# cv3vpl-lab/cylinder-pose-estimation

Hardware: AMD Instinct MI355X
Metric: frames/sec (grid-detect + cylinder fit) on 1920x1200 batch (higher is better)
Workload: dtype f64

## Files before the change

cylinder-pose-estimation_amd/csrc/masks.hip:

```cpp
#include "cpe_dev.h"

namespace cpe {

namespace {

struct W3 { unsigned long long a, b, c; };
template <int K> __device__ __forceinline__ W3 w3_up(const W3 &v, unsigned long long fill)
{
    W3 r;
    r.a = (v.a >> K) | (v.b << (64 - K));
    r.b = (v.b >> K) | (v.c << (64 - K));
    r.c = (v.c >> K) | (fill << (64 - K));
    return r;
}
template <int K> __device__ __forceinline__ W3 w3_down(const W3 &v, unsigned long long fill)
{
    W3 r;
    r.c = (v.c << K) | (v.b >> (64 - K));
    r.b = (v.b << K) | (v.a >> (64 - K));
    r.a = (v.a << K) | (fill >> (64 - K));
    return r;
}
__device__ __forceinline__ W3 w3_and(const W3 &x, const W3 &y) { return W3{x.a & y.a, x.b & y.b, x.c & y.c}; }
__device__ __forceinline__ W3 w3_or(const W3 &x, const W3 &y) { return W3{x.a | y.a, x.b | y.b, x.c | y.c}; }
// ... 921 lines not shown
{
    const int f = blockIdx.y;
    if (st[f].status != CPE_ST_OK) return;
    __shared__ unsigned long long s_win[BW_ROWS * 64];
    __shared__ float s_pts[SEG_LPW][2 * MAXVS];
    const int ncomp = min(*root_counter(st[f], list), MAXROOTS);
    if (threadIdx.x >= SEG_LPW) return;
    for (int k = blockIdx.x * SEG_LPW + threadIdx.x; k < ncomp; k += gridDim.x * SEG_LPW) {
    const int root = roots[(size_t)f * MAXROOTS + k];
    if (!comp_is_external(outside + f * plane_words, w, root, window_rect(st, f, WIN_REGION, h, w).x0)) continue;
    BitWin nz{bit_plane(base_bits, f, h, w), w, h, s_win + threadIdx.x};
    float *pts = s_pts[threadIdx.x];
    SegVisitor sv{pts, MAXVS};
    if (!trace_border(nz, root % w, root / w, false, sv, 8 * (w + h) + (1 << 20))) { set_overflow(st[f], OVF_TRACE); continue; }
    const int n = sv.n;
    if (n < MINV || n > MAXVS) continue;
    float mx = 0, my = 0;
    for (int i = 0; i < n; i++) { mx += pts[2 * i]; my += pts[2 * i + 1]; }
    mx = mx / (float)n; my = my / (float)n;
    double ax = 0, ay = 0;
    for (int i = 0; i < n; i++) { ax += (double)(pts[2 * i] - mx); ay += (double)(pts[2 * i + 1] - my); }
    ax /= n; ay /= n;
    double sxx = 0, sxy = 0, syy = 0;
    for (int i = 0; i < n; i++) {
        double dx = (double)(pts[2 * i] - mx) - ax, dy = (double)(pts[2 * i + 1] - my) - ay;
        sxx += dx * dx; sxy += dx * dy; syy += dy * dy;
    }
    double fct = 1.0 / (n - 1);
    sxx *= fct; sxy *= fct; syy *= fct;
    double wv[2], V[4];
    eig2_lapack(sxx, sxy, sxy, syy, wv, V);
    int kk = wv[1] > wv[0] ? 1 : 0;
    double ux = V[0 + kk], uy = V[2 + kk];
    int imin = 0, imax = 0;
    double pmin = 0, pmax = 0;
    for (int i = 0; i < n; i++) {
        double pr = (double)(pts[2 * i] - mx) * ux + (double)(pts[2 * i + 1] - my) * uy;
        if (i == 0 || pr < pmin) { pmin = pr; imin = i; }
        if (i == 0 || pr > pmax) { pmax = pr; imax = i; }
    }
    float p1x = pts[2 * imin], p1y = pts[2 * imin + 1], p2x = pts[2 * imax], p2y = pts[2 * imax + 1];
    float dx = p2x - p1x, dy = p2y - p1y;
    float length = (float)hypot((double)dx, (double)dy);
    if (length < 1e-8) continue;
    float at = (float)atan2((double)dy, (double)dx);
    float deg = at * (float)(180.0 / 3.14159265358979323846);
    int q = atomicAdd(&st[f].n_seg[which], 1);
    if (q >= MAXSEG) { set_overflow(st[f], OVF_SEGS); continue; }
    SegRec &r = segs[(size_t)f * MAXSEG + q];
    r.p1x = p1x; r.p1y = p1y; r.p2x = p2x; r.p2y = p2y; r.angle = -deg; r.len = length; r.valid = 1;
    }
}

__global__ __launch_bounds__(256) void k_seg_global(FrameState *__restrict__ st, int which, const SegRec *__restrict__ segs)
{
    const int f = blockIdx.x, t = threadIdx.x;
    __shared__ float s_lo, s_hi;
    __shared__ unsigned int s_len;
    const int nv = min(st[f].n_seg[which], MAXSEG);
    const SegRec *S = segs + (size_t)f * MAXSEG;
    if (t == 0) { s_lo = 0; s_hi = 0; s_len = 0; }
    __syncthreads();
    const int k_hi = nv / 2, k_lo = (nv & 1) ? nv / 2 : nv / 2 - 1;
    for (int i = t; i < nv; i += 256) {
        float ai = S[i].angle;
        int rank = 0;
        for (int j = 0; j < nv; j++) {
            float aj = S[j].angle;
            rank += (aj < ai || (aj == ai && j < i)) ? 1 : 0;
        }
        if (rank == k_lo) s_lo = ai;
        if (rank == k_hi) s_hi = ai;
        atomicMax(&s_len, __float_as_uint(S[i].len));
    }
    __syncthreads();
    if (t == 0) {
        st[f].gang[which] = (nv & 1) ? s_hi : (float)(((double)s_lo + (double)s_hi) / 2.0);
        st[f].glen[which] = __uint_as_float(s_len);
    }
}

constexpr int EXP_MAXKS = 176;
constexpr int EXP_MAXKS_PLANE = 208;
template <int MAXKS>
__global__ __launch_bounds__(256) void k_seg_expand(const uint8_t *__restrict__ base, int h, int w, int which,
                                                    FrameState *__restrict__ st, const SegRec *__restrict__ segs,
                                                    uint8_t *__restrict__ exp, int fixed_ks)
{
    constexpr int EXP_REG = 15 + MAXKS + 2;
    __shared__ uint8_t dil[EXP_REG * EXP_REG];
    __shared__ short koff[4096][2];
    __shared__ short ppix[225][2];
    __shared__ int s_nk, s_np;
    const int f = blockIdx.y, t = threadIdx.x;
    FrameState &S = st[f];
    if (S.status != CPE_ST_OK) return;
    const int njobs = 2 * min(S.n_seg[which], MAXSEG);
    for (int job = blockIdx.x; job < njobs; job += gridDim.x) {
    const int seg = job >> 1, e = job & 1;
    const SegRec r = segs[(size_t)f * MAXSEG + seg];
    const float glen = S.glen[which], gang = S.gang[which];
    if ((double)r.len > 0.8 * (double)glen) continue;
    const int ks = fixed_ks > 0 ? fixed_ks : 91 + S.r0;
    if (ks > MAXKS) { if (t == 0) set_overflow(S, OVF_KERNEL); return; }
    __syncthreads();
    const float ak = fabsf(r.angle - gang) > 5.0f ? gang : r.angle;
    const int a = ks / 2, half = 7;
    const size_t N = (size_t)h * w;
    const uint8_t *bm = base + f * N;
    const int cx = (int)rint((double)(e ? r.p2x : r.p1x)), cy = (int)rint((double)(e ? r.p2y : r.p1y));
    const int x1 = max(cx - half, 0), x2 = min(cx + half + 1, w), y1 = max(cy - half, 0), y2 = min(cy + half + 1, h);
    if (t == 0) { s_nk = 0; s_np = 0; }
    __syncthreads();
    {
        const int c = ks / 2;
        double ar = (double)ak * 3.1415926535897932384626433832795 / 180.0;
        double alpha = cos(ar), beta = sin(ar);
        double M[6] = {alpha, beta, (1 - alpha) * c - beta * c, -beta, alpha, beta * c + (1 - alpha) * c};
        double D = M[0] * M[4] - M[1] * M[3];
        D = D != 0 ? 1. / D : 0;
        double A11 = M[4] * D, A22 = M[0] * D;
        double iM[6];
        iM[0] = A11; iM[1] = M[1] * (-D); iM[3] = M[3] * (-D); iM[4] = A22;
        double b1 = -iM[0] * M[2] - iM[1] * M[5];
        double b2 = -iM[3] * M[2] - iM[4] * M[5];
        iM[2] = b1; iM[5] = b2;
        for (int i = t; i < ks * ks; i += 256) {
            int y = i / ks, x = i - y * ks;
            int X0 = (int)rint((iM[1] * y + iM[2]) * 1024) + 512;
            int Y0 = (int)rint((iM[4] * y + iM[5]) * 1024) + 512;
            int adelta = (int)rint(iM[0] * x * 1024), bdelta = (int)rint(iM[3] * x * 1024);
            int X = (X0 + adelta) >> 10, Y = (Y0 + bdelta) >> 10;
            if (X >= 0 && X < ks && Y == c) {
                int q = atomicAdd(&s_nk, 1);
                if (q < 4096) { koff[q][0] = (short)(x - a); koff[q][1] = (short)(y - a); }
            }
        }
    }
    for (int i = t; i < 225; i += 256) {
        int py = y1 + i / 15, px = x1 + i % 15;
        if (py < y2 && px < x2 && bm[(size_t)py * w + px]) {
            int q = atomicAdd(&s_np, 1);
            ppix[q][0] = (short)px; ppix[q][1] = (short)py;
        }
    }
    const int bx1 = x1 - a - 1, by1 = y1 - a - 1;
    const int bw = (x2 - x1) + 2 * a + 2, bh = (y2 - y1) + 2 * a + 2;
    for (int i = t; i < bw * bh; i += 256) dil[i] = 0;
    __syncthreads();
    const int nk = min(s_nk, 4096), np = s_np;
    if (s_nk > 4096 && t == 0) set_overflow(S, OVF_EXPAND);
    for (int i = t; i < nk * np; i += 256) {
        int p = i / nk, k = i - p * nk;
        int xx = ppix[p][0] - koff[k][0], yy = ppix[p][1] - koff[k][1];
        if (xx >= 0 && xx < w && yy >= 0 && yy < h) dil[(yy - by1) * bw + (xx - bx1)] = 1;
    }
    __syncthreads();
    uint8_t *ex = exp + f * N;
    for (int i = t; i < bw * bh; i += 256) {
        int ly = i / bw, lx = i - ly * bw;
        int gy = by1 + ly, gx = bx1 + lx;
        if (gx < 0 || gx >= w || gy < 0 || gy >= h) continue;
        bool all = true;
        for (int dy = -1; dy <= 1 && all; dy++)
            for (int dx = -1; dx <= 1; dx++) {
                int yy = gy + dy, xx = gx + dx;
                if (yy < 0 || yy >= h || xx < 0 || xx >= w) continue;
                int ly2 = ly + dy, lx2 = lx + dx;
                bool v = (ly2 >= 0 && ly2 < bh && lx2 >= 0 && lx2 < bw) ? dil[ly2 * bw + lx2] != 0 : false;
                if (!v) { all = false; break; }
            }
        if (all) ex[(size_t)gy * w + gx] = 255;
    }
    }
}

__global__ void k_masks_reset(FrameState *st, int n)
{
    int f = blockIdx.x * blockDim.x + threadIdx.x;
    if (f >= n) return;
    FrameState &S = st[f];
    S.n_joints = 0; S.n_joints_all = 0; S.n_seg[0] = 0; S.n_seg[1] = 0;
    S.gang[0] = S.gang[1] = 0; S.glen[0] = S.glen[1] = 0;
    if (S.status == CPE_ST_NO_REGION) { S.r0 = 0; S.spot[0] = S.spot[1] = S.spot[2] = S.spot[3] = 0; }
    else if (S.status == CPE_ST_OK && S.spot_fail) S.status = CPE_ST_NO_SPOT;
}

inline unsigned grid1(size_t total) { return (unsigned)((total + 255) / 256); }

}


__global__ __launch_bounds__(256) void k_blur7_bgr(const uint8_t *__restrict__ bgr, int h, int w, int tiles_x, int tiles_y, Taps t,
                                                   const FrameState *__restrict__ st, uint8_t *__restrict__ dst)
{
    constexpr int R = 3, IW = BT_X + 2 * R, IH = BT_Y + 2 * R, PER = BT_X * BT_Y / 256;
    __shared__ uint8_t s_in[IH * IW];
    __shared__ uint16_t s_h[IH * BT_X];
    const int tid = threadIdx.x;
    const int tiles = tiles_x * tiles_y;
    const int f = blockIdx.x / tiles, tt = blockIdx.x - f * tiles;
    const int gx0 = (tt % tiles_x) * BT_X, gy0 = (tt / tiles_x) * BT_Y;
    const size_t N = (size_t)h * w;
    const FrameState &S = st[f];
    if (S.status != CPE_ST_OK) return;
    int half = (int)(S.r0 / 5.0);
    if (half < 3) half = 3;
    if (half > 10) half = half + 5;
    half = max(half, (int)(S.r0 / 4.5));
    const int m = half + 1;
    if (gx0 > S.rect[0] + S.rect[2] + m || gx0 + BT_X < S.rect[0] - m || gy0 > S.rect[1] + S.rect[3] + m || gy0 + BT_Y < S.rect[1] - m)
        return;
    const uint8_t *im = bgr + f * N * 3;
    uint32_t ch[PER][3];
    for (int c = 0; c < 3; c++) {
        for (int i = tid; i < IH * IW; i += 256) {
            int ry = i / IW, rx = i - ry * IW;
            s_in[i] = im[((size_t)reflect101(gy0 - R + ry, h) * w + reflect101(gx0 - R + rx, w)) * 3 + c];
        }
        __syncthreads();
        for (int i = tid; i < IH * BT_X; i += 256) {
            int ry = i / BT_X, rx = i - ry * BT_X;
            const uint8_t *p = &s_in[ry * IW + rx];
            int sacc = 0;
#pragma unroll
            for (int j = 0; j <= 2 * R; j++) sacc += t.k[j] * p[j];
            s_h[i] = (uint16_t)sacc;
        }
        __syncthreads();
#pragma unroll
        for (int q = 0; q < PER; q++) {
            const int i = tid + q * 256;
            int ry = i / BT_X, rx = i - ry * BT_X;
            const uint16_t *p = &s_h[ry * BT_X + rx];
            int sacc = 0;
#pragma unroll
            for (int j = 0; j <= 2 * R; j++) sacc += t.k[j] * (int)p[j * BT_X];
            ch[q][c] = (uint32_t)((sacc + (1 << (t.shift - 1))) >> t.shift);
        }
        __syncthreads();
    }
#pragma unroll
    for (int q = 0; q < PER; q++) {
        const int i = tid + q * 256;
        int ry = i / BT_X, rx = i - ry * BT_X;
        if (gy0 + ry < h && gx0 + rx < w)
            dst[f * N + (size_t)(gy0 + ry) * w + gx0 + rx] = (uint8_t)((ch[q][0] * 3735u + ch[q][1] * 19235u + ch[q][2] * 9798u + 16384u) >> 15);
    }
}

int blur7_bgr(const uint8_t *bgr, int n, int h, int w, const FrameState *st, uint8_t *dst, hipStream_t s)
{
    Taps t7 = {{2, 7, 14, 18, 14, 7, 2}, 3, 12};
    CPE_LAUNCH_BEGIN();
    const int tiles_x = (w + BT_X - 1) / BT_X, tiles_y = (h + BT_Y - 1) / BT_Y;
// ... 24 lines not shown
        if (lds64 <= 96 * 1024) {
            const int bands = (h + 63) / 64;
            CPE_KLAUNCH(k_open20_joints<64>, dim3((unsigned)(n * bands)), dim3(256), lds64, s, (const uint8_t *)B.binary, h, w, bands,
                        B.hmask, B.vmask, B.joints_mask, B.jbits);
        } else {
            CPE_CHECK_ARG(lds32 <= 160 * 1024, "joints_mask_stage: frame too wide (%d columns)", w);
            const int bands = (h + 31) / 32;
            CPE_KLAUNCH(k_open20_joints<32>, dim3((unsigned)(n * bands)), dim3(256), lds32, s, (const uint8_t *)B.binary, h, w, bands,
                        B.hmask, B.vmask, B.joints_mask, B.jbits);
        }
    }
    CPE_CHECK_LAUNCH("joints_mask_stage");
    int rc;
    if ((rc = ccl_components(B.joints_mask, B.jbits, n, h, w, 0, WIN_FRAME, B.lab_p, B.roots_p, ROOTS_JOINTS, st, s)) != CPE_OK) return rc;
    const size_t fl_words = (size_t)h * ((w + 63) / 64);
    return outside_flood(B.joints_mask, n, h, w, st, WIN_FRAME, B.fl_j, B.fl_j + (size_t)n * fl_words, fl_words, s, B.jbits);
}

int spot_stage(const uint8_t *gray, int n, int h, int w, const MaskBuffers &B, FrameState *st, hipStream_t s, int planar)
{
    const size_t total = (size_t)h * w * n;
    int rc;
    CPE_LAUNCH_BEGIN();
    Taps t19 = {{1, 1, 3, 5, 10, 15, 20, 27, 30, 32, 30, 27, 20, 15, 10, 5, 3, 1, 1}, 9, 16};
    {
        const int tiles_x = (w + BT_X - 1) / BT_X, tiles_y = (h + BT_Y - 1) / BT_Y;
        CPE_CHECK_ARG(tiles_x <= 128 && (size_t)tiles_x * tiles_y <= (size_t)MAXROOTS * sizeof(int), "spot_stage: frame too large");
        uint8_t *flags = reinterpret_cast<uint8_t *>(B.roots_s);
        const size_t fstride = (size_t)MAXROOTS * sizeof(int);
        CPE_KLAUNCH(k_spot_scan, dim3((unsigned)(n * tiles_y)), dim3(256), 0, s, gray, h, w, tiles_x, tiles_y, st, flags, fstride);
        CPE_KLAUNCH(k_blur19_spot, dim3((unsigned)(n * tiles_y)), dim3(256), 0, s, gray, h, w, tiles_x, tiles_y, t19,
                    (const uint8_t *)flags, fstride, B.g19);
    }
    if ((rc = ccl_components(B.g19, nullptr, n, h, w, 240, WIN_SPOT, B.lab_s, B.roots_s, ROOTS_SPOT, st, s)) != CPE_OK) return rc;
    CPE_KLAUNCH(k_spot_area, dim3(4, n), dim3(64), 0, s, B.g19, h, w, B.roots_s, st, B.best_s);
    (void)hipMemsetAsync(B.cm, 255, total, s);
    CPE_KLAUNCH(k_spot_ellipse, dim3(n), dim3(64), 0, s, B.g19, n, h, w, B.best_s, st, B.verts, B.cm, planar);
    CPE_CHECK_LAUNCH("spot_stage");
    return CPE_OK;
}

int masks_stage(const uint8_t *gray, int n, int h, int w, const MaskBuffers &B, FrameState *st, hipStream_t s,
                const RegionSide *side, int planar, hipStream_t sj)
{
    const size_t total = (size_t)h * w * n;
    int rc;
    CPE_LAUNCH_BEGIN();
    CPE_KLAUNCH(k_masks_reset, dim3((n + 63) / 64), dim3(64), 0, s, st, n);
    const size_t fl_words = bit_plane_words(h, w);
    auto fl_plane = [&](int k) { return bit_plane(B.bits, (size_t)(2 + k) * n, h, w); };
    const bool jside = side && sj != s;
    if (jside) { (void)hipEventRecord(side->clahe_done, s); (void)hipStreamWaitEvent(sj, side->clahe_done, 0); }
    {
        hipStream_t q = jside ? sj : s;
        CPE_KLAUNCH(k_joint_centroids, dim3(frame_waves(n, 16, MAXROOTS / 64), n), dim3(64), 0, q, (const uint32_t *)B.jbits, h, w, B.roots_p, st, B.jtmp,
                    (const unsigned long long *)(B.fl_j + (size_t)n * h * ((w + 63) / 64)), (size_t)h * ((w + 63) / 64));
        CPE_KLAUNCH(k_joint_sort, dim3(n), dim3(256), 0, q, st, B.jtmp, B.joints);
    }
    const int rb_bands = (h + RB_R - 1) / RB_R;
    const size_t rb_lds = (size_t)2 * RB_ROWS * ((w + 63) / 64) * 8;
    CPE_CHECK_ARG(rb_lds <= 160 * 1024, "masks_stage: frame too wide (%d columns)", w);
    CPE_CHECK_HIP(hipFuncSetAttribute(reinterpret_cast<const void *>(&k_roi_base), hipFuncAttributeMaxDynamicSharedMemorySize, 160 * 1024));
    if (side) { (void)hipEventRecord(side->clahe_done, s); (void)hipStreamWaitEvent(side->s, side->clahe_done, 0); }
    for (int which = 0; which < 2; which++) {
        hipStream_t q = (which && side) ? side->s : s;
        const uint8_t *lm = which ? B.vmask : B.hmask;
        uint8_t *roi = which ? B.roi_v : B.roi_h;
        uint8_t *base = which ? B.base_v : B.base_h;
        uint8_t *exp = which ? B.exp_v : B.exp_h;
        uint8_t *tmp = which ? B.tmpA : B.tmpB;
        int *lab = which ? B.lab_s : B.lab, *roots = which ? B.roots_s : B.roots;
        const RootList list = which ? ROOTS_SPOT : ROOTS_MAIN;
        uint32_t *bits = reinterpret_cast<uint32_t *>(bit_plane(B.bits, which ? (size_t)n : 0, h, w));
        SegRec *segs = B.segs + (size_t)which * n * MAXSEG;
        CPE_KLAUNCH(k_roi_base, dim3((unsigned)(n * rb_bands)), dim3(256), rb_lds, q, lm, (const uint8_t *)B.cm, (const uint8_t *)B.mc,
                    h, w, rb_bands, (const FrameState *)st, roi, base, bits);
        if ((rc = ccl_components(base, bits, n, h, w, 0, WIN_REGION, lab, roots, list, st, q)) != CPE_OK) return rc;
        unsigned long long *fl_bg = fl_plane(2 + 2 * which), *fl_out = fl_plane(3 + 2 * which);
        if ((rc = outside_flood(base, n, h, w, st, WIN_REGION, fl_bg, fl_out, fl_words, q, bits)) != CPE_OK) return rc;
        if (planar) CPE_KLAUNCH((k_seg_trace<8, 700>), dim3(frame_waves(n, 32, 512), n), dim3(64), 0, q, (const uint32_t *)bits, h, w, which, (const int *)roots, list, st, segs, (const unsigned long long *)fl_out, fl_words);
        else CPE_KLAUNCH((k_seg_trace<5, 200>), dim3(frame_waves(n, 32, 512), n), dim3(64), 0, q, (const uint32_t *)bits, h, w, which, (const int *)roots, list, st, segs, (const unsigned long long *)fl_out, fl_words);
        CPE_KLAUNCH(k_seg_global, dim3(n), dim3(256), 0, q, st, which, (const SegRec *)segs);
        (void)hipMemsetAsync(tmp, 0, total, q);
        if (planar) CPE_KLAUNCH(k_seg_expand<EXP_MAXKS_PLANE>, dim3(frame_waves(n, 32, 256), n), dim3(256), 0, q, (const uint8_t *)base, h, w, which, st, (const SegRec *)segs, tmp, 201);
        else CPE_KLAUNCH(k_seg_expand<EXP_MAXKS>, dim3(frame_waves(n, 32, 256), n), dim3(256), 0, q, (const uint8_t *)base, h, w, which, st, (const SegRec *)segs, tmp, 0);
        CPE_KLAUNCH(k_or_and, dim3((unsigned)(((size_t)h * w + 16383) / 16384), n), dim3(256), 0, q, (const uint8_t *)tmp, (const uint8_t *)base,
                    (const uint8_t *)B.mc, h, w, (const FrameState *)st, exp);
        CPE_CHECK_LAUNCH("masks_stage expand");
        if ((rc = ccl_unions(exp, n, h, w, WIN_REGION, which ? B.lab_v : B.lab_h, st, q)) != CPE_OK) return rc;
    }
    if (side) { (void)hipEventRecord(side->traced, side->s); (void)hipStreamWaitEvent(s, side->traced, 0); }
    return CPE_OK;
}

}
```

cylinder-pose-estimation_amd/csrc/region.hip:

```cpp
#include "cpe_dev.h"
#include <stdlib.h>

namespace cpe {

namespace {

__constant__ uint8_t c_lab_l[256] = { 0, 1, 1, 2, 2, 3, 5, 5, 6, 7, 7, 8, 9, 9, 10, 11, 12, 12, 14, 15, 16, 17, 18, 19, 21, 23, 24, 25, 27, 27, 28, 30, 31, 33, 34, 35, 36, 38, 39, 40, 41, 42, 43, 45, 46, 47, 48, 50, 51, 52, 53, 54, 55, 57, 58, 59, 60, 61, 62, 63, 65, 66, 67, 68, 69, 70, 71, 73, 74, 75, 76, 77, 78, 79, 80, 82, 82, 83, 85, 86, 87, 88, 89, 90, 91, 92, 93, 94, 95, 97, 98, 99, 100, 101, 102, 103, 104, 105, 106, 107, 108, 109, 110, 111, 112, 113, 114, 115, 116, 117, 119, 119, 121, 122, 123, 124, 125, 126, 127, 128, 129, 130, 131, 132, 133, 134, 135, 136, 137, 138, 139, 140, 141, 142, 143, 144, 145, 146, 147, 148, 149, 150, 151, 152, 153, 154, 155, 156, 156, 157, 158, 159, 160, 161, 162, 163, 164, 165, 166, 167, 168, 169, 170, 171, 172, 173, 174, 175, 176, 177, 178, 179, 180, 180, 181, 182, 183, 184, 185, 186, 187, 188, 189, 190, 191, 192, 193, 194, 195, 196, 196, 197, 198, 199, 200, 201, 202, 203, 204, 205, 206, 207, 208, 208, 209, 210, 211, 212, 213, 214, 215, 216, 217, 218, 219, 219, 220, 221, 222, 223, 224, 225, 226, 227, 228, 228, 229, 230, 231, 232, 233, 234, 235, 236, 237, 237, 238, 239, 240, 241, 242, 243, 244, 245, 245, 246, 247, 248, 249, 250, 251, 252, 253, 253, 254, 255 };

__device__ __forceinline__ int sat_u8(int v) { return v < 0 ? 0 : (v > 255 ? 255 : v); }

struct ClaheGeom { int tilesX, tilesY, tw, th, eh, ew, clipLimit; float lutScale; };

constexpr int HIST_COPIES = 4;
__global__ __launch_bounds__(256) void k_clahe_hist(const uint8_t *__restrict__ gray, int n, int h, int w, ClaheGeom g,
                                                    int strips, unsigned int *__restrict__ hist, int lab_lut)
{
    __shared__ unsigned int sh[4 * 256 * HIST_COPIES];
    int b = blockIdx.x;
    int strip = b % strips; b /= strips;
    int tile = b % (g.tilesX * g.tilesY);
    int f = b / (g.tilesX * g.tilesY);
    int ty = tile / g.tilesX, tx = tile - ty * g.tilesX;
    for (int k = threadIdx.x; k < 4 * 256 * HIST_COPIES; k += 256) sh[k] = 0;
    __syncthreads();
// ... 557 lines not shown
}

constexpr int SEL_CAP = 256;
template <class Get>
__device__ double wave_select(Get get, int n, int k, int lane, double *s_buf , int *s_hist , int *s_cnt)
{
    double lo = -1e300, hi = 1e300;
    for (;;) {
        double mn = 1e300, mx = -1e300;
        int cnt = 0, below = 0;
        for (int i = lane; i < n; i += 64) {
            const double v = get(i);
            if (v < lo) below++;
            else if (v <= hi) { cnt++; mn = fmin(mn, v); mx = fmax(mx, v); }
        }
        for (int off = 32; off >= 1; off >>= 1) {
            mn = fmin(mn, __shfl_xor(mn, off, 64)); mx = fmax(mx, __shfl_xor(mx, off, 64));
            cnt += __shfl_xor(cnt, off, 64); below += __shfl_xor(below, off, 64);
        }
        const int kk = k - below;
        if (mx == mn) return mn;
        __syncthreads();
        if (cnt <= SEL_CAP) {
            if (lane == 0) *s_cnt = 0;
            __syncthreads();
            for (int i = lane; i < n; i += 64) {
                const double v = get(i);
                if (v >= lo && v <= hi) s_buf[atomicAdd(s_cnt, 1)] = v;
            }
            __syncthreads();
            double found = -1e300;
            for (int j = lane; j < cnt; j += 64) {
                const double x = s_buf[j];
                int less = 0, leq = 0;
                for (int q = 0; q < cnt; q++) { const double y = s_buf[q]; less += (y < x) ? 1 : 0; leq += (y <= x) ? 1 : 0; }
                if (less <= kk && kk < leq) found = x;
            }
            for (int off = 32; off >= 1; off >>= 1) found = fmax(found, __shfl_xor(found, off, 64));
            return found;
        }
        const double scale = 64.0 / (mx - mn);
        s_hist[lane] = 0;
        __syncthreads();
        for (int i = lane; i < n; i += 64) {
            const double v = get(i);
            if (v >= lo && v <= hi) atomicAdd(&s_hist[min(63, (int)((v - mn) * scale))], 1);
        }
        __syncthreads();
        const int hc = s_hist[lane];
        int incl = hc;
        for (int off = 1; off < 64; off <<= 1) { int tt = __shfl_up(incl, off, 64); if (lane >= off) incl += tt; }
        const int bstar = __popcll(__ballot(incl <= kk));
        double nlo = 1e300, nhi = -1e300;
        for (int i = lane; i < n; i += 64) {
            const double v = get(i);
            if (v >= lo && v <= hi && min(63, (int)((v - mn) * scale)) == bstar) { nlo = fmin(nlo, v); nhi = fmax(nhi, v); }
        }
        for (int off = 32; off >= 1; off >>= 1) { nlo = fmin(nlo, __shfl_xor(nlo, off, 64)); nhi = fmax(nhi, __shfl_xor(nhi, off, 64)); }
        lo = nlo; hi = nhi;
    }
}

template <class Get>
__device__ double wave_median(Get get, int n, int lane, double *s_buf, int *s_hist, int *s_cnt)
{
    const int k1 = (n - 1) / 2, k2 = n / 2;
    const double v1 = wave_select(get, n, k1, lane, s_buf, s_hist, s_cnt);
    double v2 = v1;
    if (k2 != k1) {
        int le = 0;
        double nxt = 1e300;
        for (int i = lane; i < n; i += 64) {
            const double v = get(i);
            if (v <= v1) le++;
            else nxt = fmin(nxt, v);
        }
        for (int off = 32; off >= 1; off >>= 1) { le += __shfl_xor(le, off, 64); nxt = fmin(nxt, __shfl_xor(nxt, off, 64)); }
        if (le <= k2) v2 = nxt;
    }
    return (v1 + v2) / 2.;
}

constexpr int MED_FAST = CH_DIRECT * CH_PTS;

__global__ __launch_bounds__(64) void k_blob_median(int part, int *__restrict__ sw, BlobRec *__restrict__ blobs_all,
                                                    const int *__restrict__ blob_d_all, double *__restrict__ dists_all,
                                                    const uint32_t *__restrict__ pool_all,
                                                    const unsigned short *__restrict__ blob_ch_all, FrameState *__restrict__ st,
                                                    int maxch, int maxdf)
{
    __shared__ double s_d[MED_FAST > SEL_CAP ? MED_FAST : SEL_CAP];
    __shared__ int s_ch[MAXCHAIN];
    __shared__ int s_hist[64];
    __shared__ int s_cnt;
    const int f = blockIdx.y, slot = blockIdx.z, lane = threadIdx.x;
    int *S = sw + (size_t)f * SW_STRIDE;
    const int nb = min(S[SW_NB + slot], MAXB);
    if (!part && blockIdx.x == 0 && lane == 0) S[SW_NA + slot] = nb;
    BlobRec *blobs = blobs_all + ((size_t)f * NTHR + slot) * MAXB;
    const int *blob_d = blob_d_all + ((size_t)f * NTHR + slot) * MAXB * 2;
    double *dists = dists_all + (size_t)f * NTHR * maxdf;
    const uint32_t *pool = pool_all + ((size_t)f * NTHR + slot) * maxch * 32;
    const unsigned short *blob_ch = blob_ch_all + ((size_t)f * NTHR + slot) * MAXB * CH_DIRECT;
    for (int bi = (part ? S[SW_NA + slot] : 0) + blockIdx.x; bi < nb; bi += gridDim.x) {
        const int code = blob_d[bi * 2], n = blob_d[bi * 2 + 1];
        if (code < 0 || n <= 0) continue;
        double r;
        if ((code & PTS_STORED) && n <= MED_FAST) {
            const double cx = blobs[bi].x, cy = blobs[bi].y;
            const int myid = lane < CH_DIRECT ? (int)blob_ch[bi * CH_DIRECT + lane] : 0;
            double v[MED_FAST / 64 + 1];
            double mn = 1e300, mx = -1.0;
#pragma unroll
            for (int m = 0; m < MED_FAST / 64 + 1; m++) {
                const int i = lane + 64 * m;
                const bool valid = i < n;
                const int c = __shfl(myid, valid ? i / CH_PTS : 0, 64);
                v[m] = -1.0;
                if (valid) {
                    const uint32_t p = pool[(size_t)c * 32 + i % CH_PTS];
                    const double dx = cx - (double)(int)(p & 0xFFFFu), dy = cy - (double)(int)(p >> 16);
                    v[m] = dx * dx + dy * dy;
                    mn = fmin(mn, v[m]); mx = fmax(mx, v[m]);
                }
            }
            for (int off = 32; off >= 1; off >>= 1) { mn = fmin(mn, __shfl_xor(mn, off, 64)); mx = fmax(mx, __shfl_xor(mx, off, 64)); }
            double res[2] = {mn, mn};
            if (mx > mn) {
                const double scale = 64.0 / (mx - mn);
                int bkt[MED_FAST / 64 + 1];
                __syncthreads();
                s_hist[lane] = 0;
                __syncthreads();
#pragma unroll
                for (int m = 0; m < MED_FAST / 64 + 1; m++) {
                    bkt[m] = -1;
                    if (v[m] >= 0.0) { bkt[m] = min(63, (int)((v[m] - mn) * scale)); atomicAdd(&s_hist[bkt[m]], 1); }
                }
                __syncthreads();
                const int hc = s_hist[lane];
                int incl = hc;
                for (int off = 1; off < 64; off <<= 1) { int tt = __shfl_up(incl, off, 64); if (lane >= off) incl += tt; }
                const int ks[2] = {(n - 1) / 2, n / 2};
                for (int which = 0; which < 2; which++) {
                    if (which == 1 && ks[1] == ks[0]) { res[1] = res[0]; break; }
                    const int k = ks[which];
                    const int bstar = __popcll(__ballot(incl <= k));
                    const int kk = k - __shfl(incl - hc, bstar, 64);
                    const int sz = __shfl(hc, bstar, 64);
                    __syncthreads();
                    if (lane == 0) s_cnt = 0;
                    __syncthreads();
#pragma unroll
                    for (int m = 0; m < MED_FAST / 64 + 1; m++)
                        if (bkt[m] == bstar) s_d[atomicAdd(&s_cnt, 1)] = v[m];
                    __syncthreads();
                    double found = -1.0;
                    for (int j = lane; j < sz; j += 64) {
                        const double x = s_d[j];
                        int less = 0, leq = 0;
                        for (int q = 0; q < sz; q++) { const double y = s_d[q]; less += (y < x) ? 1 : 0; leq += (y <= x) ? 1 : 0; }
                        if (less <= kk && kk < leq) found = x;
                    }
                    for (int off = 32; off >= 1; off >>= 1) found = fmax(found, __shfl_xor(found, off, 64));
                    res[which] = found;
                }
            }
            r = (sqrt(res[0]) + sqrt(res[1])) / 2.;
        } else if (code & PTS_STORED) {
            const int nch = (n + CH_PTS - 1) / CH_PTS;
            __syncthreads();
            if (lane == 0) {
                int c = code & (PTS_STORED - 1);
                for (int j = nch - 1; j >= 0; j--) { s_ch[j] = c; c = (int)pool[(size_t)c * 32 + 31]; }
            }
            __syncthreads();
            const double cx = blobs[bi].x, cy = blobs[bi].y;
            auto get = [&](int i) {
                const uint32_t p = pool[(size_t)s_ch[i / CH_PTS] * 32 + i % CH_PTS];
                const double dx = cx - (double)(int)(p & 0xFFFFu), dy = cy - (double)(int)(p >> 16);
                return sqrt(dx * dx + dy * dy);
            };
            r = wave_median(get, n, lane, s_d, s_hist, &s_cnt);
        } else {
            const double *dd = dists + code;
            r = wave_median([&](int i) { return dd[i]; }, n, lane, s_d, s_hist, &s_cnt);
        }
        if (lane == 0) blobs[bi].r = r;
    }
}

__device__ __forceinline__ bool blob_joins(double gx, double gy, double gr, double cx, double cy, double cr)
{
    const double dx = gx - cx, dy = gy - cy;
    const double d2 = dx * dx + dy * dy;
    const double a = fmax(fmax(10.0, gr), cr);
    if (d2 >= a * a * 1.0000000000009095) return false;
    const double dist = sqrt(d2);
    const bool isNew = dist >= 10.0 && dist >= gr && dist >= cr;
    return !isNew;
}

__device__ __forceinline__ int wave_min_int(int v)
{
    for (int off = 32; off >= 1; off >>= 1) v = min(v, __shfl_xor(v, off, 64));
    return v;
}

constexpr int MG_NT = 256;
constexpr int MG_CELLS = 1024;
constexpr int MG_LCAP = 24;
constexpr int MG_STAGE = MG_LCAP - 4;
constexpr int MG_RANK_DIRECT = 4096, MG_RANK_BUCKETS = 4096;
__global__ __launch_bounds__(MG_NT) void k_blob_merge(FrameState *__restrict__ st, const int *__restrict__ sw,
                                                    const BlobRec *__restrict__ blobs_all, int *__restrict__ order,
                                                    Group *__restrict__ groups, int always_replay, double *__restrict__ gmid_all,
                                                    int h, int w)
{
    __shared__ double sX[MAXG_LDS], sY[MAXG_LDS], sR[MAXG_LDS];
    __shared__ int s_next[MAXG_LDS];
    __shared__ unsigned char s_gn[MAXG_LDS];
    __shared__ int s_head[MG_CELLS];
    __shared__ double s_maxr;
    __shared__ double bX[64], bY[64], bR[64];
    __shared__ double pl[MG_LCAP * 3][64];
    __shared__ double cX[64], cY[64], cR[64];
    __shared__ int cG[64], s_bad[64];
    __shared__ int pn[64], pg[64], pd[64], s_jm[64], s_mod[64];
    __shared__ int s_ng, s_serial, s_adv, s_maxn;
    const int f = blockIdx.x, t = threadIdx.x, lane = t & 63;
    FrameState &S = st[f];
    int *ord = order + (size_t)f * 2 * MAXB;
    Group *G = groups + (size_t)f * MAXG;
    double *gm = gmid_all + (size_t)f * (MAXG - MAXG_LDS) * 4 - (size_t)MAXG_LDS * 4;
    auto gm_load = [&](int j, int k) { return __hip_atomic_load(gm + 4 * (size_t)j + k, __ATOMIC_RELAXED, __HIP_MEMORY_SCOPE_AGENT); };
    auto mid_joins = [&](int j, double cx, double cy, double cr) {
        if (j < MAXG_LDS) return blob_joins(sX[j], sY[j], sR[j], cx, cy, cr);
        return blob_joins(gm_load(j, 0), gm_load(j, 1), gm_load(j, 2), cx, cy, cr);
    };
    auto mid_set = [&](int j, double x, double y, double r) {
        if (j < MAXG_LDS) { sX[j] = x; sY[j] = y; sR[j] = r; }
        else { gm[4 * (size_t)j] = x; gm[4 * (size_t)j + 1] = y; gm[4 * (size_t)j + 2] = r; }
    };
    int cs = 64;
    while (((w + cs - 1) / cs) * ((h + cs - 1) / cs) > MG_CELLS) cs *= 2;
    const int gw = (w + cs - 1) / cs, gh = (h + cs - 1) / cs;
    const double inv_cs = 1.0 / cs;
    auto cell_x = [&](double x) { return min(max((int)floor(x * inv_cs), 0), gw - 1); };
    auto cell_y = [&](double y) { return min(max((int)floor(y * inv_cs), 0), gh - 1); };
    auto cell_of = [&](double x, double y) { return cell_y(y) * gw + cell_x(x); };
    auto mid_cell = [&](int j) { return j < MAXG_LDS ? cell_of(sX[j], sY[j]) : cell_of(gm_load(j, 0), gm_load(j, 1)); };
    auto nxt_get = [&](int j) { return j < MAXG_LDS ? s_next[j] : (int)gm_load(j, 3); };
    auto nxt_set = [&](int j, int v) { if (j < MAXG_LDS) s_next[j] = v; else gm[4 * (size_t)j + 3] = (double)v; };
    auto grid_link = [&](int j, int c) { nxt_set(j, atomicExch(&s_head[c], j)); };
    auto grid_unlink = [&](int j, int c) {
        int p = s_head[c];
        if (p == j) { s_head[c] = nxt_get(j); return; }
        for (int it = 0; p >= 0 && it < MAXG; it++) {
            const int q = nxt_get(p);
            if (q == j) { nxt_set(p, nxt_get(j)); return; }
            p = q;
        }
    };
    auto grid_first = [&](double cx, double cy, double cr, int limit, int part, int nsplit) {
        const double R = fmax(fmax(10.0, cr), s_maxr) + 1.0;
        const int x0 = cell_x(cx - R), x1 = cell_x(cx + R), y0 = cell_y(cy - R), y1 = cell_y(cy + R);
        int first = INT_MAX, k = 0;
        for (int yy = y0; yy <= y1; yy++)
            for (int xx = x0; xx <= x1; xx++, k++) {
                if (k % nsplit != part) continue;
                int it = 0;
// ... 1363 lines not shown
```

Before: 3626.

## Bit-pack segment expansion and register-resident blob median selection

Segment expansion now builds the rotated line kernel as per-row intervals found by binary search and dilates with 64-bit row words and atomicOr, then erodes with word-level shifts. One 64-thread block handles both segment endpoints, replacing 256-thread byte-array work. Separately, the blob median for small stored blobs runs a register-only iterative bucket select using ballots, picks a template size by point count, and prefetches the next blob's descriptors. This cuts shared-memory traffic and synchronisation but adds considerable complexity and risk of subtle mismatches with the original rasterisation.

```diff
diff --git a/cylinder-pose-estimation_amd/csrc/masks.hip b/cylinder-pose-estimation_amd/csrc/masks.hip
--- a/cylinder-pose-estimation_amd/csrc/masks.hip
+++ b/cylinder-pose-estimation_amd/csrc/masks.hip
@@ -1027,36 +1027,40 @@
 
 constexpr int EXP_MAXKS = 176;
 constexpr int EXP_MAXKS_PLANE = 208;
+constexpr int EXP_WPR = 4;
+__device__ __forceinline__ unsigned long long exp_range_mask(int wd, int lo, int hi)
+{
+    const int a = max(lo - 64 * wd, 0), b = min(hi - 64 * wd, 64);
+    if (a >= b) return 0ull;
+    const unsigned long long upto_b = b >= 64 ? ~0ull : ((1ull << b) - 1ull);
+    return upto_b & ~((1ull << a) - 1ull);
+}
 template <int MAXKS>
-__global__ __launch_bounds__(256) void k_seg_expand(const uint8_t *__restrict__ base, int h, int w, int which,
-                                                    FrameState *__restrict__ st, const SegRec *__restrict__ segs,
-                                                    uint8_t *__restrict__ exp, int fixed_ks)
+__global__ __launch_bounds__(64) void k_seg_expand(const uint8_t *__restrict__ base, int h, int w, int which,
+                                                   FrameState *__restrict__ st, const SegRec *__restrict__ segs,
+                                                   uint8_t *__restrict__ exp, int fixed_ks)
 {
     constexpr int EXP_REG = 15 + MAXKS + 2;
-    __shared__ uint8_t dil[EXP_REG * EXP_REG];
-    __shared__ short koff[4096][2];
-    __shared__ short ppix[225][2];
-    __shared__ int s_nk, s_np;
-    const int f = blockIdx.y, t = threadIdx.x;
+    static_assert(EXP_REG < 64 * EXP_WPR, "the support box and one column beyond it fit the row words");
+    __shared__ unsigned long long dil[(EXP_REG + 2) * EXP_WPR];
+    __shared__ short s_iv[MAXKS][2];
+    __shared__ unsigned int s_prow[16];
+    const int f = blockIdx.y, lane = threadIdx.x;
     FrameState &S = st[f];
     if (S.status != CPE_ST_OK) return;
-    const int njobs = 2 * min(S.n_seg[which], MAXSEG);
-    for (int job = blockIdx.x; job < njobs; job += gridDim.x) {
-    const int seg = job >> 1, e = job & 1;
+    const int nseg = min(S.n_seg[which], MAXSEG);
+    for (int seg = blockIdx.x; seg < nseg; seg += gridDim.x) {
     const SegRec r = segs[(size_t)f * MAXSEG + seg];
     const float glen = S.glen[which], gang = S.gang[which];
     if ((double)r.len > 0.8 * (double)glen) continue;
     const int ks = fixed_ks > 0 ? fixed_ks : 91 + S.r0;
-    if (ks > MAXKS) { if (t == 0) set_overflow(S, OVF_KERNEL); return; }
+    if (ks > MAXKS) { if (lane == 0) set_overflow(S, OVF_KERNEL); return; }
     __syncthreads();
     const float ak = fabsf(r.angle - gang) > 5.0f ? gang : r.angle;
     const int a = ks / 2, half = 7;
     const size_t N = (size_t)h * w;
     const uint8_t *bm = base + f * N;
-    const int cx = (int)rint((double)(e ? r.p2x : r.p1x)), cy = (int)rint((double)(e ? r.p2y : r.p1y));
-    const int x1 = max(cx - half, 0), x2 = min(cx + half + 1, w), y1 = max(cy - half, 0), y2 = min(cy + half + 1, h);
-    if (t == 0) { s_nk = 0; s_np = 0; }
-    __syncthreads();
+    bool major_x;
     {
         const int c = ks / 2;
         double ar = (double)ak * 3.1415926535897932384626433832795 / 180.0;
@@ -1070,52 +1074,99 @@
         double b1 = -iM[0] * M[2] - iM[1] * M[5];
         double b2 = -iM[3] * M[2] - iM[4] * M[5];
         iM[2] = b1; iM[5] = b2;
-        for (int i = t; i < ks * ks; i += 256) {
-            int y = i / ks, x = i - y * ks;
+        auto srcX = [&](int x, int y) {
             int X0 = (int)rint((iM[1] * y + iM[2]) * 1024) + 512;
+            int adelta = (int)rint(iM[0] * x * 1024);
+            return (X0 + adelta) >> 10;
+        };
+        auto srcY = [&](int x, int y) {
             int Y0 = (int)rint((iM[4] * y + iM[5]) * 1024) + 512;
-            int adelta = (int)rint(iM[0] * x * 1024), bdelta = (int)rint(iM[3] * x * 1024);
-            int X = (X0 + adelta) >> 10, Y = (Y0 + bdelta) >> 10;
-            if (X >= 0 && X < ks && Y == c) {
-                int q = atomicAdd(&s_nk, 1);
-                if (q < 4096) { koff[q][0] = (short)(x - a); koff[q][1] = (short)(y - a); }
+            int bdelta = (int)rint(iM[3] * x * 1024);
+            return (Y0 + bdelta) >> 10;
+        };
+        major_x = fabs(iM[4]) >= fabs(iM[3]);
+        const bool incY = (major_x ? iM[4] : iM[3]) >= 0, incX = (major_x ? iM[1] : iM[0]) >= 0;
+        int nk = 0;
+        for (int u = lane; u < ks; u += 64) {
+            auto below = [&](auto g, bool inc, int target) {
+                int lo = 0, hi = ks;
+                while (lo < hi) {
+                    const int mid = (lo + hi) >> 1, v = inc ? mid : ks - 1 - mid;
+                    if (g(v) >= target) hi = mid; else lo = mid + 1;
+                }
+                return lo;
+            };
+            auto gY = [&](int v) { return major_x ? srcY(u, v) : srcY(v, u); };
+            auto gX = [&](int v) { return major_x ? srcX(u, v) : srcX(v, u); };
+            const int y_a = below(gY, incY, c), y_b = below(gY, incY, c + 1);
+            const int x_a = below(gX, incX, 0), x_b = below(gX, incX, ks);
+            const int ylo = incY ? y_a : ks - y_b, yhi = incY ? y_b - 1 : ks - 1 - y_a;
+            const int xlo = incX ? x_a : ks - x_b, xhi = incX ? x_b - 1 : ks - 1 - x_a;
+            const int lo = max(ylo, xlo), hi = min(yhi, xhi);
+            s_iv[u][0] = (short)lo; s_iv[u][1] = (short)hi;
+            nk += max(hi - lo + 1, 0);
+        }
+        for (int off = 32; off >= 1; off >>= 1) nk += __shfl_xor(nk, off, 64);
+        if (nk > 4096 && lane == 0) set_overflow(S, OVF_EXPAND);
+    }
+    uint8_t *ex = exp + f * N;
+    for (int e = 0; e < 2; e++) {
+        const int cx = (int)rint((double)(e ? r.p2x : r.p1x)), cy = (int)rint((double)(e ? r.p2y : r.p1y));
+        const int x1 = max(cx - half, 0), x2 = min(cx + half + 1, w), y1 = max(cy - half, 0), y2 = min(cy + half + 1, h);
+        __syncthreads();
+        unsigned int prow = 0;
+        if (lane < 15) {
+            const int py = y1 + lane;
+            if (py < y2)
+                for (int j = 0; j < 15; j++)
+                    if (x1 + j < x2 && bm[(size_t)py * w + x1 + j]) prow |= 1u << j;
+            s_prow[lane] = prow;
+        }
+        if (__ballot(prow != 0) == 0ull) continue;
+        const int bx1 = x1 - a - 1, by1 = y1 - a - 1;
+        const int bw = (x2 - x1) + 2 * a + 2, bh = (y2 - y1) + 2 * a + 2;
+        for (int i = lane; i < (bh + 2) * EXP_WPR; i += 64) dil[i] = 0ull;
+        __syncthreads();
+        for (int i = lane; i < ks * 15; i += 64) {
+            const int u = i / 15, pr = i - u * 15;
+            const unsigned long long bits = s_prow[pr];
+            if (!bits) continue;
+            const int lo = s_iv[u][0], hi = s_iv[u][1];
+            for (int v = lo; v <= hi; v++) {
+                const int x = major_x ? u : v, y = major_x ? v : u;
+                const int ly = pr + 1 + 2 * a - y, lx = 1 + 2 * a - x;
+                unsigned long long *row = dil + (ly + 1) * EXP_WPR;
+                const int wd = lx >> 6, sh = lx & 63;
+                atomicOr(row + wd, bits << sh);
+                if (sh > 49) atomicOr(row + wd + 1, bits >> (64 - sh));
             }
         }
-    }
-    for (int i = t; i < 225; i += 256) {
-        int py = y1 + i / 15, px = x1 + i % 15;
-        if (py < y2 && px < x2 && bm[(size_t)py * w + px]) {
-            int q = atomicAdd(&s_np, 1);
-            ppix[q][0] = (short)px; ppix[q][1] = (short)py;
-        }
-    }
-    const int bx1 = x1 - a - 1, by1 = y1 - a - 1;
-    const int bw = (x2 - x1) + 2 * a + 2, bh = (y2 - y1) + 2 * a + 2;
-    for (int i = t; i < bw * bh; i += 256) dil[i] = 0;
-    __syncthreads();
-    const int nk = min(s_nk, 4096), np = s_np;
-    if (s_nk > 4096 && t == 0) set_overflow(S, OVF_EXPAND);
-    for (int i = t; i < nk * np; i += 256) {
-        int p = i / nk, k = i - p * nk;
-        int xx = ppix[p][0] - koff[k][0], yy = ppix[p][1] - koff[k][1];
-        if (xx >= 0 && xx < w && yy >= 0 && yy < h) dil[(yy - by1) * bw + (xx - bx1)] = 1;
-    }
-    __syncthreads();
-    uint8_t *ex = exp + f * N;
-    for (int i = t; i < bw * bh; i += 256) {
-        int ly = i / bw, lx = i - ly * bw;
-        int gy = by1 + ly, gx = bx1 + lx;
-        if (gx < 0 || gx >= w || gy < 0 || gy >= h) continue;
-        bool all = true;
-        for (int dy = -1; dy <= 1 && all; dy++)
-            for (int dx = -1; dx <= 1; dx++) {
-                int yy = gy + dy, xx = gx + dx;
-                if (yy < 0 || yy >= h || xx < 0 || xx >= w) continue;
-                int ly2 = ly + dy, lx2 = lx + dx;
-                bool v = (ly2 >= 0 && ly2 < bh && lx2 >= 0 && lx2 < bw) ? dil[ly2 * bw + lx2] != 0 : false;
-                if (!v) { all = false; break; }
+        __syncthreads();
+        const int in_lo = max(-bx1, 0), in_hi = min(w - bx1, 64 * EXP_WPR);
+        for (int i = lane; i < (bh + 2) * EXP_WPR; i += 64) {
+            const int ly = (i >> 2) - 1, wd = i & 3, gy = by1 + ly;
+            const unsigned long long in = exp_range_mask(wd, in_lo, in_hi);
+            dil[i] = (gy < 0 || gy >= h) ? ~0ull : ((dil[i] & in) | ~in);
+        }
+        __syncthreads();
+        for (int i = lane; i < bh * EXP_WPR; i += 64) {
+            const int ly = i >> 2, wd = i & 3, gy = by1 + ly;
+            if (gy < 0 || gy >= h) continue;
+            unsigned long long er = exp_range_mask(wd, in_lo, min(in_hi, bw));
+            if (!er) continue;
+            for (int dy = 0; dy < 3; dy++) {
+                const unsigned long long *row = dil + (ly + dy) * EXP_WPR;
+                const unsigned long long pc = row[wd];
+                const unsigned long long pm = wd > 0 ? row[wd - 1] >> 63 : ((bx1 < 1 || gy + dy < 1 || gy + dy > h) ? 1ull : 0ull);
+                const unsigned long long pn = wd < EXP_WPR - 1 ? row[wd + 1] << 63 : 0ull;
+                er &= pc & ((pc << 1) | pm) & ((pc >> 1) | pn);
             }
-        if (all) ex[(size_t)gy * w + gx] = 255;
+            const long long o = (long long)gy * w + bx1 + 64 * wd;
+            while (er) {
+                ex[o + __ffsll((long long)er) - 1] = 255;
+                er &= er - 1;
+            }
+        }
     }
     }
 }
@@ -1306,8 +1357,8 @@
         else CPE_KLAUNCH((k_seg_trace<5, 200>), dim3(frame_waves(n, 32, 512), n), dim3(64), 0, q, (const uint32_t *)bits, h, w, which, (const int *)roots, list, st, segs, (const unsigned long long *)fl_out, fl_words);
         CPE_KLAUNCH(k_seg_global, dim3(n), dim3(256), 0, q, st, which, (const SegRec *)segs);
         (void)hipMemsetAsync(tmp, 0, total, q);
-        if (planar) CPE_KLAUNCH(k_seg_expand<EXP_MAXKS_PLANE>, dim3(frame_waves(n, 32, 256), n), dim3(256), 0, q, (const uint8_t *)base, h, w, which, st, (const SegRec *)segs, tmp, 201);
-        else CPE_KLAUNCH(k_seg_expand<EXP_MAXKS>, dim3(frame_waves(n, 32, 256), n), dim3(256), 0, q, (const uint8_t *)base, h, w, which, st, (const SegRec *)segs, tmp, 0);
+        if (planar) CPE_KLAUNCH(k_seg_expand<EXP_MAXKS_PLANE>, dim3(frame_waves(n, 32, 256), n), dim3(64), 0, q, (const uint8_t *)base, h, w, which, st, (const SegRec *)segs, tmp, 201);
+        else CPE_KLAUNCH(k_seg_expand<EXP_MAXKS>, dim3(frame_waves(n, 32, 256), n), dim3(64), 0, q, (const uint8_t *)base, h, w, which, st, (const SegRec *)segs, tmp, 0);
         CPE_KLAUNCH(k_or_and, dim3((unsigned)(((size_t)h * w + 16383) / 16384), n), dim3(256), 0, q, (const uint8_t *)tmp, (const uint8_t *)base,
                     (const uint8_t *)B.mc, h, w, (const FrameState *)st, exp);
         CPE_CHECK_LAUNCH("masks_stage expand");
diff --git a/cylinder-pose-estimation_amd/csrc/region.hip b/cylinder-pose-estimation_amd/csrc/region.hip
--- a/cylinder-pose-estimation_amd/csrc/region.hip
+++ b/cylinder-pose-estimation_amd/csrc/region.hip
@@ -663,6 +663,90 @@
 }
 
 constexpr int MED_FAST = CH_DIRECT * CH_PTS;
+constexpr int MED_DIRECT = 12;
+
+__device__ __forceinline__ double wave_read_lane(double x, int src)
+{
+    return __hiloint2double(__builtin_amdgcn_readlane(__double2hiint(x), src), __builtin_amdgcn_readlane(__double2loint(x), src));
+}
+
+template <int M>
+__device__ __forceinline__ double blob_radius_regs(const uint32_t *__restrict__ pool, int myid, double cx, double cy, int n, int lane)
+{
+    constexpr double NONE = 1e300;
+    double v[M];
+    double mn = NONE, mx = -1.0;
+#pragma unroll
+    for (int m = 0; m < M; m++) {
+        const int i = lane + 64 * m;
+        const bool valid = i < n;
+        const int c = __shfl(myid, valid ? i / CH_PTS : 0, 64);
+        v[m] = NONE;
+        if (valid) {
+            const uint32_t p = pool[(size_t)c * 32 + i % CH_PTS];
+            const double dx = cx - (double)(int)(p & 0xFFFFu), dy = cy - (double)(int)(p >> 16);
+            v[m] = dx * dx + dy * dy;
+            mn = fmin(mn, v[m]); mx = fmax(mx, v[m]);
+        }
+    }
+    for (int off = 32; off >= 1; off >>= 1) { mn = fmin(mn, __shfl_xor(mn, off, 64)); mx = fmax(mx, __shfl_xor(mx, off, 64)); }
+    const int k1 = (n - 1) / 2, k2 = n / 2;
+    double lo = mn, hi = mx, v1 = mn;
+    while (hi > lo) {
+        const double scale = 64.0 / (hi - lo);
+        int bkt[M];
+#pragma unroll
+        for (int m = 0; m < M; m++) bkt[m] = v[m] < lo ? -1 : (v[m] <= hi ? min(63, (int)((v[m] - lo) * scale)) : 64);
+        int b = 0;
+#pragma unroll
+        for (int step = 32; step >= 1; step >>= 1) {
+            int before = 0;
+#pragma unroll
+            for (int m = 0; m < M; m++) before += __popcll(__ballot(bkt[m] < b + step));
+            if (before <= k1) b += step;
+        }
+        int sz = 0;
+#pragma unroll
+        for (int m = 0; m < M; m++) sz += __popcll(__ballot(bkt[m] == b));
+        if (sz <= MED_DIRECT) {
+            bool found = false;
+#pragma unroll
+            for (int m = 0; m < M; m++) {
+                unsigned long long members = __ballot(bkt[m] == b);
+                while (members && !found) {
+                    const double x = wave_read_lane(v[m], __ffsll((long long)members) - 1);
+                    int less = 0, leq = 0;
+#pragma unroll
+                    for (int q = 0; q < M; q++) { less += __popcll(__ballot(v[q] < x)); leq += __popcll(__ballot(v[q] <= x)); }
+                    if (less <= k1 && k1 < leq) { v1 = x; found = true; }
+                    members &= ~__ballot(v[m] == x);
+                }
+            }
+            break;
+        }
+        double nlo = NONE, nhi = -1.0;
+#pragma unroll
+        for (int m = 0; m < M; m++)
+            if (bkt[m] == b) { nlo = fmin(nlo, v[m]); nhi = fmax(nhi, v[m]); }
+        for (int off = 32; off >= 1; off >>= 1) { nlo = fmin(nlo, __shfl_xor(nlo, off, 64)); nhi = fmax(nhi, __shfl_xor(nhi, off, 64)); }
+        lo = nlo; hi = nhi; v1 = nlo;
+    }
+    double v2 = v1;
+    if (k2 != k1) {
+        int leq = 0;
+#pragma unroll
+        for (int m = 0; m < M; m++) leq += __popcll(__ballot(v[m] <= v1));
+        if (leq <= k2) {
+            double nxt = NONE;
+#pragma unroll
+            for (int m = 0; m < M; m++)
+                if (v[m] > v1) nxt = fmin(nxt, v[m]);
+            for (int off = 32; off >= 1; off >>= 1) nxt = fmin(nxt, __shfl_xor(nxt, off, 64));
+            v2 = nxt;
+        }
+    }
+    return (sqrt(v1) + sqrt(v2)) / 2.;
+}
 
 __global__ __launch_bounds__(64) void k_blob_median(int part, int *__restrict__ sw, BlobRec *__restrict__ blobs_all,
                                                     const int *__restrict__ blob_d_all, double *__restrict__ dists_all,
@@ -670,7 +754,7 @@
                                                     const unsigned short *__restrict__ blob_ch_all, FrameState *__restrict__ st,
                                                     int maxch, int maxdf)
 {
-    __shared__ double s_d[MED_FAST > SEL_CAP ? MED_FAST : SEL_CAP];
+    __shared__ double s_d[SEL_CAP];
     __shared__ int s_ch[MAXCHAIN];
     __shared__ int s_hist[64];
     __shared__ int s_cnt;
@@ -679,95 +763,57 @@
     const int nb = min(S[SW_NB + slot], MAXB);
     if (!part && blockIdx.x == 0 && lane == 0) S[SW_NA + slot] = nb;
     BlobRec *blobs = blobs_all + ((size_t)f * NTHR + slot) * MAXB;
-    const int *blob_d = blob_d_all + ((size_t)f * NTHR + slot) * MAXB * 2;
+    const int2 *blob_d = reinterpret_cast<const int2 *>(blob_d_all) + ((size_t)f * NTHR + slot) * MAXB;
     double *dists = dists_all + (size_t)f * NTHR * maxdf;
     const uint32_t *pool = pool_all + ((size_t)f * NTHR + slot) * maxch * 32;
     const unsigned short *blob_ch = blob_ch_all + ((size_t)f * NTHR + slot) * MAXB * CH_DIRECT;
-    for (int bi = (part ? S[SW_NA + slot] : 0) + blockIdx.x; bi < nb; bi += gridDim.x) {
-        const int code = blob_d[bi * 2], n = blob_d[bi * 2 + 1];
-        if (code < 0 || n <= 0) continue;
-        double r;
-        if ((code & PTS_STORED) && n <= MED_FAST) {
-            const double cx = blobs[bi].x, cy = blobs[bi].y;
-            const int myid = lane < CH_DIRECT ? (int)blob_ch[bi * CH_DIRECT + lane] : 0;
-            double v[MED_FAST / 64 + 1];
-            double mn = 1e300, mx = -1.0;
-#pragma unroll
-            for (int m = 0; m < MED_FAST / 64 + 1; m++) {
-                const int i = lane + 64 * m;
-                const bool valid = i < n;
-                const int c = __shfl(myid, valid ? i / CH_PTS : 0, 64);
-                v[m] = -1.0;
-                if (valid) {
-                    const uint32_t p = pool[(size_t)c * 32 + i % CH_PTS];
-                    const double dx = cx - (double)(int)(p & 0xFFFFu), dy = cy - (double)(int)(p >> 16);
-                    v[m] = dx * dx + dy * dy;
-                    mn = fmin(mn, v[m]); mx = fmax(mx, v[m]);
-                }
-            }
-            for (int off = 32; off >= 1; off >>= 1) { mn = fmin(mn, __shfl_xor(mn, off, 64)); mx = fmax(mx, __shfl_xor(mx, off, 64)); }
-            double res[2] = {mn, mn};
-            if (mx > mn) {
-                const double scale = 64.0 / (mx - mn);
-                int bkt[MED_FAST / 64 + 1];
+    int bi = (part ? S[SW_NA + slot] : 0) + blockIdx.x;
+    if (bi >= nb) return;
+    int2 dn = blob_d[bi];
+    double cx = blobs[bi].x, cy = blobs[bi].y;
+    int myid = lane < CH_DIRECT ? (int)blob_ch[bi * CH_DIRECT + lane] : 0;
+    for (;;) {
+        const int bn = bi + gridDim.x;
+        const bool more = bn < nb;
+        int2 ndn = make_int2(-1, 0);
+        double ncx = 0, ncy = 0;
+        int nid = 0;
+        if (more) {
+            ndn = blob_d[bn];
+            ncx = blobs[bn].x; ncy = blobs[bn].y;
+            nid = lane < CH_DIRECT ? (int)blob_ch[bn * CH_DIRECT + lane] : 0;
+        }
+        const int code = __builtin_amdgcn_readfirstlane(dn.x), n = __builtin_amdgcn_readfirstlane(dn.y);
+        if (code >= 0 && n > 0) {
+            double r;
+            if ((code & PTS_STORED) && n <= MED_FAST) {
+                if (n <= 64) r = blob_radius_regs<1>(pool, myid, cx, cy, n, lane);
+                else if (n <= 128) r = blob_radius_regs<2>(pool, myid, cx, cy, n, lane);
+                else if (n <= 192) r = blob_radius_regs<3>(pool, myid, cx, cy, n, lane);
+                else if (n <= 256) r = blob_radius_regs<4>(pool, myid, cx, cy, n, lane);
+                else r = blob_radius_regs<MED_FAST / 64 + 1>(pool, myid, cx, cy, n, lane);
+            } else if (code & PTS_STORED) {
+                const int nch = (n + CH_PTS - 1) / CH_PTS;
                 __syncthreads();
-                s_hist[lane] = 0;
-                __syncthreads();
-#pragma unroll
-                for (int m = 0; m < MED_FAST / 64 + 1; m++) {
-                    bkt[m] = -1;
-                    if (v[m] >= 0.0) { bkt[m] = min(63, (int)((v[m] - mn) * scale)); atomicAdd(&s_hist[bkt[m]], 1); }
+                if (lane == 0) {
+                    int c = code & (PTS_STORED - 1);
+                    for (int j = nch - 1; j >= 0; j--) { s_ch[j] = c; c = (int)pool[(size_t)c * 32 + 31]; }
                 }
                 __syncthreads();
-                const int hc = s_hist[lane];
-                int incl = hc;
-                for (int off = 1; off < 64; off <<= 1) { int tt = __shfl_up(incl, off, 64); if (lane >= off) incl += tt; }
-                const int ks[2] = {(n - 1) / 2, n / 2};
-                for (int which = 0; which < 2; which++) {
-                    if (which == 1 && ks[1] == ks[0]) { res[1] = res[0]; break; }
-                    const int k = ks[which];
-                    const int bstar = __popcll(__ballot(incl <= k));
-                    const int kk = k - __shfl(incl - hc, bstar, 64);
-                    const int sz = __shfl(hc, bstar, 64);
-                    __syncthreads();
-                    if (lane == 0) s_cnt = 0;
-                    __syncthreads();
-#pragma unroll
-                    for (int m = 0; m < MED_FAST / 64 + 1; m++)
-                        if (bkt[m] == bstar) s_d[atomicAdd(&s_cnt, 1)] = v[m];
-                    __syncthreads();
-                    double found = -1.0;
-                    for (int j = lane; j < sz; j += 64) {
-                        const double x = s_d[j];
-                        int less = 0, leq = 0;
-                        for (int q = 0; q < sz; q++) { const double y = s_d[q]; less += (y < x) ? 1 : 0; leq += (y <= x) ? 1 : 0; }
-                        if (less <= kk && kk < leq) found = x;
-                    }
-                    for (int off = 32; off >= 1; off >>= 1) found = fmax(found, __shfl_xor(found, off, 64));
-                    res[which] = found;
-                }
-            }
-            r = (sqrt(res[0]) + sqrt(res[1])) / 2.;
-        } else if (code & PTS_STORED) {
-            const int nch = (n + CH_PTS - 1) / CH_PTS;
-            __syncthreads();
-            if (lane == 0) {
-                int c = code & (PTS_STORED - 1);
-                for (int j = nch - 1; j >= 0; j--) { s_ch[j] = c; c = (int)pool[(size_t)c * 32 + 31]; }
-            }
-            __syncthreads();
-            const double cx = blobs[bi].x, cy = blobs[bi].y;
-            auto get = [&](int i) {
-                const uint32_t p = pool[(size_t)s_ch[i / CH_PTS] * 32 + i % CH_PTS];
-                const double dx = cx - (double)(int)(p & 0xFFFFu), dy = cy - (double)(int)(p >> 16);
-                return sqrt(dx * dx + dy * dy);
-            };
-            r = wave_median(get, n, lane, s_d, s_hist, &s_cnt);
-        } else {
-            const double *dd = dists + code;
-            r = wave_median([&](int i) { return dd[i]; }, n, lane, s_d, s_hist, &s_cnt);
-        }
-        if (lane == 0) blobs[bi].r = r;
+                auto get = [&](int i) {
+                    const uint32_t p = pool[(size_t)s_ch[i / CH_PTS] * 32 + i % CH_PTS];
+                    const double dx = cx - (double)(int)(p & 0xFFFFu), dy = cy - (double)(int)(p >> 16);
+                    return sqrt(dx * dx + dy * dy);
+                };
+                r = wave_median(get, n, lane, s_d, s_hist, &s_cnt);
+            } else {
+                const double *dd = dists + code;
+                r = wave_median([&](int i) { return dd[i]; }, n, lane, s_d, s_hist, &s_cnt);
+            }
+            if (lane == 0) blobs[bi].r = r;
+        }
+        if (!more) break;
+        bi = bn; dn = ndn; cx = ncx; cy = ncy; myid = nid;
     }
 }
 
```

Measured after the change: 3728 (median of 6 runs). 1.03x the previous value.
